# wolny/pytorch-3dunet

Measured on AMD Instinct MI355X. Metric: volumetric patches/sec (fwd+bwd), UNet3D f_maps=32 patch 64x128x128, higher is better.
Workload: dtype f32

## Files before the change

### pytorch-3dunet_amd/csrc/u3d_bf16.hip

```cpp
#include "u3d_common.h"
#include "u3d_gn.h"
#include <type_traits>

typedef __bf16 bf16x8 __attribute__((ext_vector_type(8)));
typedef __bf16 bf16x4 __attribute__((ext_vector_type(4)));
typedef __bf16 bf16x2 __attribute__((ext_vector_type(2)));
typedef float f32x2 __attribute__((ext_vector_type(2)));
typedef unsigned u32x4 __attribute__((ext_vector_type(4)));
typedef unsigned u32x2 __attribute__((ext_vector_type(2)));

__device__ __forceinline__ bf16x8 u3d_stage_b16(const bf16x8& v, bool has_aff, bool ok, const f32x4& a0, const f32x4& b0, const f32x4& a1,
                                                const f32x4& b1) {
    const u32x4 raw = __builtin_bit_cast(u32x4, v);
    u32x4 o = raw;
    if (has_aff) {
#pragma unroll
        for (int e = 0; e < 4; ++e) {
            const f32x2 x = {__builtin_bit_cast(float, raw[e] << 16), __builtin_bit_cast(float, raw[e] & 0xffff0000u)};
            const f32x2 a = e < 2 ? f32x2{a0[2 * e], a0[2 * e + 1]} : f32x2{a1[2 * e - 4], a1[2 * e - 3]};
            const f32x2 b = e < 2 ? f32x2{b0[2 * e], b0[2 * e + 1]} : f32x2{b1[2 * e - 4], b1[2 * e - 3]};
            o[e] = __builtin_bit_cast(unsigned, __builtin_convertvector(__builtin_elementwise_fma(x, a, b), bf16x2));
        }
    }
    const unsigned m = ok ? 0xffffffffu : 0u;
    return __builtin_bit_cast(bf16x8, u32x4{o[0] & m, o[1] & m, o[2] & m, o[3] & m});
}

extern int g_u3d_tune[24];

namespace {

constexpr int HS = 12;

struct bf16_conv_params {
    const float* x;
    const float* affine;
    const bf16x8* wpk;
    float* y;
    const float* residual;
    const float* gx;
    double* out_stats;
    double* gstats;
    int N, D, H, W, C, K, relu;
    int tz, ty, tx;
    int off;
    const float* maskx;
    int ksplit;
    float* ws;
    long long wpart;
    int order;
    int b16;
    int t8mode, t8cs;
};

template <int ZW, int KS>
struct tile_geom {
    static constexpr bool FLAT = ZW == 3;
    static constexpr int TZ = FLAT ? 5 : 4 * ZW, TY = FLAT ? 10 : 8, TX = FLAT ? 10 : 8;
    static constexpr int HZ = TZ + KS - 1, HY = TY + KS - 1, HX = TX + KS - 1, MT = FLAT ? 4 : 2 * ZW;
    static_assert(HX <= HS, "halo rows are HS records long");
    static constexpr int NTAPS = KS * KS * KS;
    static constexpr int RING = KS == 3 ? 9 : 8;
    static constexpr int BDIST = 6;
    static constexpr int ADIST = 2;
    static constexpr int PLANE = HZ * HY * HS * 16 + 64;
    static constexpr int BUF = 2 * PLANE;
    static constexpr int ITEMS = HZ * HY * HX * 4;
    static constexpr int ITERS = (ITEMS + 255) / 256;
    static constexpr int NPARTS = KS * KS;
    static constexpr int PER_PART = (ITERS + NPARTS - 1) / NPARTS;
    static constexpr int ITEMS8 = HZ * HY * HX * 2;
    static constexpr int ITERS8 = (ITEMS8 + 255) / 256;
    static constexpr int PER_PART8 = (ITERS8 + NPARTS - 1) / NPARTS;
};

template <int NT, int ZW, int KS, typename T = float>
__device__ __forceinline__ void conv_tile_epilogue(const bf16_conv_params& p, f32x16 (&acc)[tile_geom<ZW, KS>::MT][NT], char* lds, int n, int nb,
                                                   int split, int z0, int y0, int x0, int t, int lane, int w) {
    using G = tile_geom<ZW, KS>;
    const int col = lane & 31, half = lane >> 5;
    if (p.ksplit > 1) {
// ... 2760 lines not shown
```

### pytorch-3dunet_amd/csrc/u3d_conv.hip

```cpp
#include <type_traits>
#include <utility>

#include "u3d_common.h"
#include "u3d_gn.h"
#include "u3d_subpix.h"

int g_u3d_tune[24] = {0};

namespace cv {
constexpr int TZ = 4, TY = 8, TX = 8;
constexpr int HZ = TZ + 2, HY = TY + 2, HX = TX + 2;
constexpr int CC = 16;
constexpr int CS = 16;
constexpr int RS = HX * CS + 4;
constexpr int PS = HY * RS;
constexpr int TILE_FLOATS = HZ * PS + 4;
constexpr int CNT_OFF = 2 * TILE_FLOATS;
constexpr int RED_OFF = CNT_OFF + 16;
constexpr int LDS_FLOATS = RED_OFF + 4 * 3 * 32 * 2;
constexpr int NITEMS = HZ * HY * HX * (CC / 4);
constexpr int NIT = (NITEMS + 255) / 256;
constexpr int NSTEP = 27 * (CC / 8);
constexpr int NSTEP_PAIRY = 36 * (CC / 8);
constexpr int NSTEP_N16 = 27;
constexpr int ST0 = 30;
constexpr int ISTORE = 5;
constexpr int PACK_PAD = 5;
static_assert(2 * (NIT - 1) < ST0 - 8 && ST0 + NIT <= NSTEP, "prefetch schedule must fit the k-loop");
}

struct ConvParams {
    u3d_src_t src;
    u3d_src_t gx;
    const float* wp;
    float* out;
    double* out_stats;
    double* gstats;
    const float* res;
    int N, D, H, W, Cout;
    int nchunks, ncb, ntot;
    int tz, ty, tx;
    int relu, vec, has_gx, ovec;
    int total;
    int gx_x2;
    int stagger;
    int stat_reps;
    int zfast;
    int ksplit, cps;
    long long part_stride;
    long long* dbg;
    int oz0, oy0, ox0, oz1, oy1, ox1;
    int mz, my, mx;
};

#define U3D_DBG_STAMP(slot)                                                   \
    do {                                                                      \
        if constexpr (DBG) {                                                  \
            if (l == 0) dbgw[slot] = (long long)__builtin_readcyclecounter(); \
        }                                                                     \
    } while (0)
// ... 1018 lines not shown
                            }
                            if (v16 == 0) {
                                double* r = &red[(((T.n & 1) * NT) * 32 + 4 * kq + e) * 2];
                                __hip_atomic_fetch_add(r, (double)a, __ATOMIC_RELAXED, __HIP_MEMORY_SCOPE_WORKGROUP);
                                __hip_atomic_fetch_add(r + 1, (double)b2, __ATOMIC_RELAXED, __HIP_MEMORY_SCOPE_WORKGROUP);
                            }
                        }
                    } else {
                        const int cq_ = (l >> 2) & 7;
                        stat_reduce(sq1, sq2, T.n, 0, PAIRY ? 4 * (cq_ & 3) : 4 * cq_);
                    }
                    sq1 = f32x4{0.f, 0.f, 0.f, 0.f};
                    sq2 = f32x4{0.f, 0.f, 0.f, 0.f};
                }
            }
            flush_stats(T.n, T.cb);
        }
        if (!has_next_tile) break;
        if constexpr (!ZEROC) {
#pragma unroll
            for (int mt = 0; mt < MT; ++mt)
#pragma unroll
                for (int nt = 0; nt < NT; ++nt)
#pragma unroll
                    for (int r = 0; r < 16; ++r) acc[mt][nt][r] = 0.f;
        }
        wi = nwi;
        dT = dTN;
        T = TN;
        wq = wqn;
    }
    if constexpr (DBG) {
        if (l == 0) dbgw[4] = ntiles;
    }
    U3D_DBG_STAMP(6);
}

namespace wg {
constexpr int TZ = 2, TY = 8, TX = 8;
constexpr int HZ = TZ + 2, HY = TY + 2, HX = TX + 2;
constexpr int CC = 32;
constexpr int CSg = 32, RSg = HX * CSg, PSg = HY * RSg;
constexpr int G_FLOATS = HZ * PSg;
constexpr int TV = TZ * TY * TX;
constexpr int DZ_FLOATS = TV * 32;
constexpr int DUMMY_OFF = G_FLOATS + DZ_FLOATS;
constexpr int BUF_FLOATS = G_FLOATS + DZ_FLOATS + 4;
constexpr int LDS_FLOATS = 2 * BUF_FLOATS;
constexpr int NTHR = 512;
constexpr int NITEMS_G = HZ * HY * HX * (CC / 4);
constexpr int NIT_G = (NITEMS_G + NTHR - 1) / NTHR;
constexpr int NIT_DZ = TV * 8 / NTHR;
constexpr int MAX_MAP_INTS = 4096;
}

struct WgradParams {
    u3d_src_t src;
    const float* dz;
    float* partial;
    int N, D, H, W, Cout;
    int nchunks, nkb, S;
    int tz, ty, tx, ntiles, tps;
    int vec, dzvec;
    int bz0, by0, bx0, bz1, by1, bx1;
};

template <bool VEC, bool REG = false, bool PAIR = false>
__global__ __launch_bounds__(512, 2) void conv3d_wgrad_kernel(const WgradParams p) {
    using namespace wg;
    constexpr int NA = PAIR ? 4 : 7;
    extern __shared__ __attribute__((aligned(16))) float lds[];
    int* zmapl = reinterpret_cast<int*>(lds + 2 * BUF_FLOATS);
    __builtin_amdgcn_s_setprio(3);
    const int t = threadIdx.x;
    const int l = t & 63, i = l & 31, h = l >> 5;
    const int w = __builtin_amdgcn_readfirstlane(t >> 6);
    const int tg = w & 3, hf = w >> 2;

    const int logical = u3d_xcd_remap(blockIdx.x, gridDim.x);
    const int kb = logical % p.nkb;
    const int chunk = (logical / p.nkb) % p.nchunks;
    const int s = logical / (p.nkb * p.nchunks);
    const int D = p.D, H = p.H, W = p.W;
    const int Ctot = p.src.C0 + p.src.C1;
    int* ymapl = zmapl + D;
    int* xmapl = ymapl + H;
    if (p.src.C1 > 0) {
        for (int k = t; k < D; k += NTHR) zmapl[k] = p.src.zmap[k];
        for (int k = t; k < H; k += NTHR) ymapl[k] = p.src.ymap[k];
        for (int k = t; k < W; k += NTHR) xmapl[k] = p.src.xmap[k];
        __syncthreads();
    }

    f32x16 acc[NA];
#pragma unroll
    for (int k = 0; k < NA; ++k)
#pragma unroll
        for (int r = 0; r < 16; ++r) acc[k][r] = 0.f;

    const int q = t & 7, tv = t >> 3;
    const int cq = chunk * CC + 4 * q;
    const int co = kb * 32 + 4 * q;
    const bool cok = cq < Ctot, from0 = cq < p.src.C0, dcok = co < p.Cout;
    const float* gbase = !cok ? p.src.p0 : (from0 ? p.src.p0 + cq : p.src.p1 + (cq - p.src.C0));
    const int Cs = (from0 || !cok) ? p.src.C0 : p.src.C1;
    const float* dzbase = p.dz + (dcok ? co : 0);

    constexpr int NPFC = NIT_G + NIT_DZ;
    int rel[NPFC], loff[NPFC];
    unsigned fz0 = 0, fz1 = 0, fy0 = 0, fy1 = 0, fx0 = 0, fx1 = 0, fdead = 0;
    if constexpr (REG) {
        const int vz = D % TZ ? D % TZ : TZ, vy = H % TY ? H % TY : TY, vx = W % TX ? W % TX : TX;
#pragma unroll
        for (int it = 0; it < NIT_G; ++it) {
            const int vox = tv + 64 * it;
            const int hz = vox / (HY * HX);
            const int rem = vox - hz * (HY * HX);
            const int hy = rem / HX;
            const int hx = rem - hy * HX;
            const bool in = vox < HZ * HY * HX;
            rel[it] = from0 ? ((hz - 1) * H + (hy - 1)) * W + (hx - 1)
                            : (((hz - 1) >> 1) * p.src.H1 + ((hy - 1) >> 1)) * p.src.W1 + ((hx - 1) >> 1);
            loff[it] = in ? hz * PSg + hy * RSg + hx * CSg + 4 * q : DUMMY_OFF;
            fz0 |= (in && hz == 0 ? 1u : 0u) << it;
            fz1 |= (in && hz > vz ? 1u : 0u) << it;
            fy0 |= (in && hy == 0 ? 1u : 0u) << it;
            fy1 |= (in && hy > vy ? 1u : 0u) << it;
            fx0 |= (in && hx == 0 ? 1u : 0u) << it;
            fx1 |= (in && hx > vx ? 1u : 0u) << it;
            fdead |= (in && cok ? 0u : 1u) << it;
        }
#pragma unroll
        for (int it = 0; it < NIT_DZ; ++it) {
            const int vox = tv + 64 * it;
            rel[NIT_G + it] = ((vox >> 6) * H + ((vox >> 3) & 7)) * W + (vox & 7);
            loff[NIT_G + it] = G_FLOATS + vox * 32 + 4 * q;
            fz1 |= ((vox >> 6) >= vz ? 1u : 0u) << (NIT_G + it);
            fy1 |= (((vox >> 3) & 7) >= vy ? 1u : 0u) << (NIT_G + it);
            fx1 |= ((vox & 7) >= vx ? 1u : 0u) << (NIT_G + it);
        }
        fdead |= (dcok ? 0u : 3u) << NIT_G;
    }
    auto tile_invalid = [&](int z0, int y0, int x0) {
        unsigned inv = fdead;
        inv |= z0 == 0 ? fz0 : 0u;
        inv |= z0 + TZ >= D ? fz1 : 0u;
        inv |= y0 == 0 ? fy0 : 0u;
        inv |= y0 + TY >= H ? fy1 : 0u;
        inv |= x0 == 0 ? fx0 : 0u;
        inv |= x0 + TX >= W ? fx1 : 0u;
        return inv;
// ... 124 lines not shown
        f32x4 ga, gb;
        u3d_load_affine(p.src.affine, c.n, Ctot, cq, false, ga, gb);
#pragma unroll 1
        for (int it = 0; it < NIT_G; ++it) {
            const int vox = tv + 64 * it;
            if (vox >= HZ * HY * HX) continue;
            const int hz = vox / (HY * HX), rem = vox - hz * (HY * HX), hy = rem / HX, hx = rem - hy * HX;
            const int gz = c.z0 - 1 + hz, gy = c.y0 - 1 + hy, gxx = c.x0 - 1 + hx;
            f32x4 val = {0.f, 0.f, 0.f, 0.f};
            if (gz >= 0 && gz < D && gy >= 0 && gy < H && gxx >= 0 && gxx < W) {
                int v0, v1;
                u3d_vox_index(p.src, c.n, gz, gy, gxx, D, H, W, v0, v1);
                val = u3d_load_quad(p.src, v0, v1, cq, false) * ga + gb;
            }
            *reinterpret_cast<f32x4*>(&buf[hz * PSg + hy * RSg + hx * CSg + 4 * q]) = val;
        }
#pragma unroll 1
        for (int it = 0; it < NIT_DZ; ++it) {
            const int vox = tv + 64 * it;
            const int z = c.z0 + (vox >> 6), y = c.y0 + ((vox >> 3) & 7), x = c.x0 + (vox & 7);
            f32x4 val = {0.f, 0.f, 0.f, 0.f};
            if (z < p.bz1 && y < p.by1 && x < p.bx1) {
                const float* sp = p.dz + ((size_t)((c.n * D + z) * H + y) * W + x) * p.Cout + co;
#pragma unroll
                for (int e = 0; e < 4; ++e)
                    if (co + e < p.Cout) val[e] = sp[e];
            }
            *reinterpret_cast<f32x4*>(&buf[G_FLOATS + vox * 32 + 4 * q]) = val;
        }
    };

    constexpr int NPF = NIT_G + NIT_DZ;
    constexpr int ST0 = 20;
    static_assert(2 * (NPF - 1) < ST0 && ST0 + NPF <= 32, "prefetch schedule must fit the 32 groups of a tile");
    const int tile_begin = s * p.tps, tile_end = min(p.ntiles, (s + 1) * p.tps);

    TileIdx tix = tile_decode(tile_begin);
    if (tile_begin < tile_end) {
        const TileC c = tile_coords(tix);
        if constexpr (VEC) {
            f32x4 ga, gb;
            load_affine(c.n, ga, gb);
            f32x4 v[NPF];
#pragma unroll
            for (int k = 0; k < NPF; ++k) v[k] = pf_load(c, k);
#pragma unroll
            for (int k = 0; k < NPF; ++k) pf_store(lds, c, k, v[k], ga, gb);
        } else {
            stage_scalar(lds, c);
        }
    }
    __syncthreads();

    int abase[NA];
#pragma unroll
    for (int k = 0; k < NA; ++k) {
        const int tap = PAIR ? 2 * (tg + 4 * k) + (i >> 4) : tg + 4 * k;
        const int toff = tap < 27 ? (tap / 9) * PSg + ((tap / 3) % 3) * RSg + (tap % 3) * CSg : 0;
        abase[k] = (PAIR ? (i & 15) : i) + h * CSg + hf * PSg + toff;
    }
    int bbase = G_FLOATS + (hf * 64 + h) * 32 + i;
    int cur = 0;
    __builtin_amdgcn_s_setprio(0);

    f32x4 gan = {1.f, 1.f, 1.f, 1.f}, gbn = {0.f, 0.f, 0.f, 0.f};
    int n_aff = -1;
    for (int tile = tile_begin; tile < tile_end; ++tile) {
        const bool has_next = tile + 1 < tile_end;
        if (has_next) tix = tile_next(tix);
        const TileC cn = tile_coords(tix);
        float* nbuf = lds + (cur ^ 1) * BUF_FLOATS;
        f32x4 v[NPF];
        if constexpr (VEC) {
            if (cn.n != n_aff) {
                load_affine(cn.n, gan, gbn);
                n_aff = cn.n;
            }
        }
        const float* gl = lds + cur * BUF_FLOATS;

        float aop[2][NA], bop[2];
        bop[0] = gl[bbase];
#pragma unroll
        for (int k = 0; k < NA; ++k) aop[0][k] = gl[abase[k]];
#pragma unroll
        for (int g = 0; g < 32; ++g) {
            if constexpr (VEC) {
                if (g % 2 == 0 && g / 2 < NPF) v[g / 2] = pf_load(cn, g / 2);
                if (g >= ST0 && g - ST0 < NPF) pf_store(nbuf, cn, g - ST0, v[g - ST0], gan, gbn);
            }
            if (g + 1 < 32) {
                const int row = (g + 1) >> 2, tq = (g + 1) & 3;
                const int goff = row * RSg + 2 * tq * CSg;
                bop[(g + 1) & 1] = gl[bbase + (row * 8 + 2 * tq) * 32];
#pragma unroll
                for (int k = 0; k < NA; ++k) aop[(g + 1) & 1][k] = gl[abase[k] + goff];
            }
            __builtin_amdgcn_sched_barrier(0);
#pragma unroll
            for (int k = 0; k < NA; ++k) acc[k] = __builtin_amdgcn_mfma_f32_32x32x2f32(aop[g & 1][k], bop[g & 1], acc[k], 0, 0, 0);
            __builtin_amdgcn_sched_barrier(0);
        }
        if constexpr (!VEC) {
            if (has_next) stage_scalar(nbuf, cn);
        }
        __syncthreads();
        cur ^= 1;
    }

    __builtin_amdgcn_s_setprio(3);
    float* red = lds;
    if (hf == 1) {
#pragma unroll
        for (int k = 0; k < NA; ++k)
#pragma unroll
            for (int r = 0; r < 16; ++r) red[((tg * 7 + k) * 16 + r) * 64 + l] = acc[k][r];
    }
    __syncthreads();
    if (hf == 0) {
        float* dst = p.partial + ((size_t)((s * p.nchunks + chunk) * p.nkb + kb) * 27) * 1024;
#pragma unroll
        for (int k = 0; k < NA; ++k) {
#pragma unroll
            for (int r = 0; r < 16; ++r) {
                const int row = (r & 3) + 8 * (r >> 2) + 4 * h;
                const int tap = PAIR ? 2 * (tg + 4 * k) + (row >> 4) : tg + 4 * k;
                const int c = PAIR ? (row & 15) : row;
                if (tap < 27) dst[((size_t)tap * 32 + c) * 32 + i] = acc[k][r] + red[((tg * 7 + k) * 16 + r) * 64 + l];
            }
        }
    }
}

template <int G>
__global__ __launch_bounds__(256) void wgrad_reduce_kernel(const float* __restrict__ partial, float* __restrict__ dw,
                                                           int S, int nchunks, int nkb, int Cin, int Cout, int cstride,
                                                           int has_job, u3d_gn_bwd_job_t job) {
    __shared__ float red[4][64];
    if (has_job && blockIdx.x == 0) {
        extern __shared__ double shb[];
        u3d_gn_bwd_finalize_body(job.gstats_lo, job.mean_rstd, job.gamma, job.N, job.C0 + job.C1, job.G, job.count, 1, 1, job.dgamma,
                                 job.dbeta, job.coef, job.gstats_hi, job.C0, job.hi_scale, job.coef_hi, shb, job.reps_lo, job.reps_hi);
        return;
    }
    const long long total = (long long)Cin * 27 * Cout;
    const int lane = G == 1 ? (int)threadIdx.x : (int)(threadIdx.x & 63), grp = G == 1 ? 0 : (int)(threadIdx.x >> 6);
    const long long idx = (long long)(blockIdx.x - (has_job ? 1 : 0)) * (G == 1 ? 256 : 64) + lane;
    float sum = 0.f;
    int k = 0, tap = 0, c = 0;
    if (idx < total) {
        k = (int)(idx % Cout);
        const long long r = idx / Cout;
        tap = (int)(r % 27);
        c = (int)(r / 27);
        const int chunk = c >> 5, kb = k >> 5;
        const size_t off = ((size_t)(chunk * nkb + kb) * 27 + tap) * 1024 + (c & 31) * 32 + (k & 31);
        const size_t sstride = (size_t)nchunks * nkb * 27 * 1024;
        const int per = (S + G - 1) / G;
        const int s0 = grp * per, s1 = min(S, s0 + per);
        float a0 = 0.f, a1 = 0.f, a2 = 0.f, a3 = 0.f;
        int s = s0;
        for (; s + 3 < s1; s += 4) {
            a0 += partial[(size_t)s * sstride + off];
            a1 += partial[(size_t)(s + 1) * sstride + off];
            a2 += partial[(size_t)(s + 2) * sstride + off];
            a3 += partial[(size_t)(s + 3) * sstride + off];
        }
        for (; s < s1; ++s) a0 += partial[(size_t)s * sstride + off];
        sum = (a0 + a1) + (a2 + a3);
    }
    if constexpr (G == 1) {
        if (idx < total) dw[((size_t)k * cstride + c) * 27 + tap] = sum;
    } else {
        red[grp][lane] = sum;
        __syncthreads();
        if (grp == 0 && idx < total)
            dw[((size_t)k * cstride + c) * 27 + tap] = (red[0][lane] + red[1][lane]) + (red[2][lane] + red[3][lane]);
    }
}

__device__ __forceinline__ int pack_image_of(long long idx, int nchunks, int ntot, long long& id) {
// ... 299 lines not shown
        v /= H;
        const int z = (int)(v % D);
        const int n = (int)(v / D);
        float sum = 0.f;
        for (int tap = 0; tap < 27; ++tap) {
            const int zz = z + tap / 9 - 1, yy = y + (tap / 3) % 3 - 1, xx = x + tap % 3 - 1;
            if (zz < 0 || zz >= D || yy < 0 || yy >= H || xx < 0 || xx >= W) continue;
            int v0, v1;
            u3d_vox_index(src, n, zz, yy, xx, D, H, W, v0, v1);
            for (int c = 0; c < Cin; ++c) {
                float g = u3d_load_elem(src, v0, v1, c);
                if (src.affine) {
                    const float* ab = src.affine + ((size_t)n * Cin + c) * 2;
                    g = g * ab[0] + ab[1];
                }
                const float wt = flip ? w[((size_t)c * Cout + co) * 27 + (26 - tap)] : w[((size_t)co * Cin + c) * 27 + tap];
                sum += g * wt;
            }
        }
        if (relu) sum = fmaxf(sum, 0.f);
        out[idx] = sum;
    }
}

static inline int cdiv(int a, int b) { return (a + b - 1) / b; }

static bool src_vec_ok(const u3d_src_t* s) {
    if (s->C0 % 4 != 0 || s->C1 % 4 != 0) return false;
    if (((uintptr_t)s->p0 & 15) != 0) return false;
    if (s->C1 > 0 && ((uintptr_t)s->p1 & 15) != 0) return false;
    if (s->affine && ((uintptr_t)s->affine & 15) != 0) return false;
    return true;
}

static int check_src(const u3d_src_t* s, const char* what) {
    U3D_REQUIRE(s != nullptr && s->p0 != nullptr && (s->C0 > 0 || s->C1 > 0) && s->C0 >= 0, "%s: null source", what);
    U3D_REQUIRE(s->C1 >= 0, "%s: negative C1", what);
    if (s->C1 > 0)
        U3D_REQUIRE(s->p1 && s->zmap && s->ymap && s->xmap && s->D1 > 0 && s->H1 > 0 && s->W1 > 0,
                    "%s: low-res source needs p1, index maps and dims", what);
    return 0;
}

static long long* g_u3d_prof_buf = nullptr;
static size_t g_u3d_prof_records = 0;

extern "C" int u3d_set_profile_buffer(void* device_buffer, size_t bytes) {
    g_u3d_prof_buf = static_cast<long long*>(device_buffer);
    g_u3d_prof_records = device_buffer ? bytes / (24 * sizeof(long long)) : 0;
    return 0;
}

extern "C" int u3d_set_tuning(int key, int value) {
    if (key < 0 || key >= 24) return u3d_set_err(U3D_EINVAL, "u3d_set_tuning: key out of range");
    g_u3d_tune[key] = value;
    return 0;
}

extern "C" size_t u3d_packed_weight_floats(int Cin, int Cout, int mode) {
    return (size_t)pack_total_floats(Cin, Cout, mode, nullptr, nullptr);
}

extern "C" int u3d_pack_weights(int device, u3d_stream_t stream, const float* w, int Cout, int Cin, int mode,
                                float* packed) {
    U3D_ENTER(device);
    U3D_REQUIRE(w && packed && Cout > 0 && Cin > 0 && (mode == 0 || mode == 1), "u3d_pack_weights: bad argument");
    int nchunks = 0, ntot = 0;
    const long long total = pack_total_floats(Cin, Cout, mode, &nchunks, &ntot);
    const int blocks = (int)((total + 255) / 256 > 4096 ? 4096 : (total + 255) / 256);
    hipLaunchKernelGGL(pack_weights_kernel, dim3(blocks), dim3(256), 0, (hipStream_t)stream, w, packed, Cout, Cin,
                       mode, nchunks, ntot, total);
    U3D_LAUNCH_CHECK();
    return 0;
}

extern "C" int u3d_pack_weights_batch(int device, u3d_stream_t stream, const u3d_pack_desc_t* descs_device, int n,
                                      int64_t total_floats) {
    U3D_ENTER(device);
    U3D_REQUIRE(descs_device && n > 0 && total_floats > 0, "u3d_pack_weights_batch: bad argument");
    U3D_REQUIRE(total_floats % 4 == 0, "u3d_pack_weights_batch: image sizes are multiples of 4 floats");
    long long blocks = (total_floats / 4 + 255) / 256;
    if (blocks > 8192) blocks = 8192;
    hipLaunchKernelGGL(pack_weights_batch_kernel, dim3((unsigned)blocks), dim3(256), 0, (hipStream_t)stream, descs_device, n,
                       (long long)total_floats);
    U3D_LAUNCH_CHECK();
    return 0;
}

extern "C" long long u3d_pack_weights_cells_blocks(const float* w, int Cin, int Cout, int mode, int cin_stride) {
    const int cs = cin_stride > 0 ? cin_stride : Cin;
    if (Cin <= 0 || Cout <= 0 || mode < 0 || mode > 3 || Cin % 4 != 0 || Cout % 4 != 0 || cs % 4 != 0 || ((uintptr_t)w & 15) != 0) return 0;
    return pack_cells_of(Cin, Cout, mode) + 1;
}

extern "C" int u3d_pack_weights_batch_cells(int device, u3d_stream_t stream, const u3d_pack_desc_t* descs_device, int n,
                                            long long total_blocks) {
    U3D_ENTER(device);
    U3D_REQUIRE(descs_device && n > 0 && total_blocks > 0 && total_blocks < 0x7fffffffLL, "u3d_pack_weights_batch_cells: bad argument");
    hipLaunchKernelGGL(pack_weights_cells_kernel, dim3((unsigned)total_blocks), dim3(256), 0, (hipStream_t)stream, descs_device, n);
    U3D_LAUNCH_CHECK();
    return 0;
}

static int device_cu_count(int device, int* out) {
    static int cached[64] = {0};
    if (device >= 0 && device < 64 && cached[device] > 0) {
        *out = cached[device];
// ... 350 lines not shown
        else                                                                                     \
            hipLaunchKernelGGL((conv3d_mfma_kernel<NT_, false>), grid, block, shmem, st, p);     \
    } while (0)
    if (nt == 3)
        U3D_CONV_LAUNCH(3);
    else if (nt == 2)
        U3D_CONV_LAUNCH(2);
    else
        U3D_CONV_LAUNCH(1);
#undef U3D_CONV_LAUNCH
    U3D_LAUNCH_CHECK();
    return 0;
}

static void wgrad_plan(int N, int D, int H, int W, int Cin, int Cout, WgradParams& p) {
    p.nchunks = cdiv(Cin, 32);
    p.nkb = cdiv(Cout, 32);
    p.tz = cdiv(D, wg::TZ), p.ty = cdiv(H, wg::TY), p.tx = cdiv(W, wg::TX);
    p.ntiles = N * p.tz * p.ty * p.tx;
    const int pairs = p.nchunks * p.nkb;
    const int ncu = 256;
    long long best_cost = -1;
    int best_S = 1;
    for (int rounds = 1; rounds <= 8; ++rounds) {
        int S = (rounds * ncu) / pairs;
        if (S < 1) S = 1;
        if (S > p.ntiles) S = p.ntiles;
        const int tps = cdiv(p.ntiles, S);
        S = cdiv(p.ntiles, tps);
        const long long cost = (long long)cdiv(S * pairs, ncu) * (tps + 2);
        if (best_cost < 0 || cost < best_cost) {
            best_cost = cost;
            best_S = S;
        }
    }
    if (g_u3d_tune[1] > 0) best_S = g_u3d_tune[1] > p.ntiles ? p.ntiles : g_u3d_tune[1];
    p.tps = cdiv(p.ntiles, best_S);
    p.S = cdiv(p.ntiles, p.tps);
}

extern "C" size_t u3d_wgrad_workspace_floats(int N, int D, int H, int W, int Cin, int Cout) {
    WgradParams p;
    wgrad_plan(N, D, H, W, Cin, Cout, p);
    return (size_t)p.S * p.nchunks * p.nkb * 27 * 1024;
}

static int wgrad_set_lds_once(int device) {
    static bool done[64] = {false};
    if (device >= 0 && device < 64 && done[device]) return 0;
    U3D_HIP(hipFuncSetAttribute(reinterpret_cast<const void*>(conv3d_wgrad_kernel<true, true>),
                                hipFuncAttributeMaxDynamicSharedMemorySize, (wg::LDS_FLOATS + wg::MAX_MAP_INTS) * sizeof(float)));
    U3D_HIP(hipFuncSetAttribute(reinterpret_cast<const void*>(conv3d_wgrad_kernel<true, true, true>),
                                hipFuncAttributeMaxDynamicSharedMemorySize, (wg::LDS_FLOATS + wg::MAX_MAP_INTS) * sizeof(float)));
    U3D_HIP(hipFuncSetAttribute(reinterpret_cast<const void*>(conv3d_wgrad_kernel<true>),
                                hipFuncAttributeMaxDynamicSharedMemorySize, (wg::LDS_FLOATS + wg::MAX_MAP_INTS) * sizeof(float)));
    U3D_HIP(hipFuncSetAttribute(reinterpret_cast<const void*>(conv3d_wgrad_kernel<false>),
                                hipFuncAttributeMaxDynamicSharedMemorySize, (wg::LDS_FLOATS + wg::MAX_MAP_INTS) * sizeof(float)));
    if (device >= 0 && device < 64) done[device] = true;
    return 0;
}

static int conv3d_wgrad_impl(int device, u3d_stream_t stream, const u3d_src_t* src, const float* dz, float* dw, int cstride,
                             int N, int D, int H, int W, int Cout, float* workspace, size_t workspace_floats, const int* box = nullptr,
                             const u3d_gn_bwd_job_t* job = nullptr);

extern "C" int u3d_conv3d_wgrad_box(int device, u3d_stream_t stream, const u3d_src_t* src, const float* dz, float* dw, int N, int D,
                                    int H, int W, int Cout, float* workspace, size_t workspace_floats, const int* box) {
    U3D_REQUIRE(box != nullptr, "u3d_conv3d_wgrad_box: box is NULL");
    return conv3d_wgrad_impl(device, stream, src, dz, dw, 0, N, D, H, W, Cout, workspace, workspace_floats, box);
}

extern "C" int u3d_conv3d_wgrad(int device, u3d_stream_t stream, const u3d_src_t* src, const float* dz, float* dw,
                                int N, int D, int H, int W, int Cout, float* workspace, size_t workspace_floats) {
    return conv3d_wgrad_impl(device, stream, src, dz, dw, 0, N, D, H, W, Cout, workspace, workspace_floats);
}

extern "C" int u3d_conv3d_wgrad_strided(int device, u3d_stream_t stream, const u3d_src_t* src, const float* dz, float* dw,
                                        int dw_cin_stride, int N, int D, int H, int W, int Cout, float* workspace,
                                        size_t workspace_floats) {
    U3D_REQUIRE(src && dw_cin_stride >= src->C0 + src->C1, "u3d_conv3d_wgrad_strided: dw_cin_stride < channels of src");
    return conv3d_wgrad_impl(device, stream, src, dz, dw, dw_cin_stride, N, D, H, W, Cout, workspace, workspace_floats);
}

static size_t wgrad_job_lds_bytes(int N, int C, int G) { return sizeof(double) * (4 * (size_t)N * C + 2 * (size_t)N * G); }

extern "C" int u3d_conv3d_wgrad_job_supported(int N, int C, int G) {
    return (N > 0 && C > 0 && G > 0 && C % G == 0 && wgrad_job_lds_bytes(N, C, G) + 1024 <= 64 * 1024) ? 1 : 0;
}

extern "C" int u3d_conv3d_wgrad_job(int device, u3d_stream_t stream, const u3d_src_t* src, const float* dz, float* dw,
                                    int dw_cin_stride, int N, int D, int H, int W, int Cout, float* workspace,
                                    size_t workspace_floats, const u3d_gn_bwd_job_t* job) {
    U3D_REQUIRE(src && (dw_cin_stride == 0 || dw_cin_stride >= src->C0 + src->C1), "u3d_conv3d_wgrad_job: dw_cin_stride < channels of src");
    if (job) {
        U3D_REQUIRE(job->gstats_lo && job->mean_rstd && job->gamma && job->dgamma && job->dbeta && job->coef && job->C0 > 0 &&
                        job->C1 >= 0 && (job->C1 == 0) == (job->gstats_hi == nullptr) && (job->coef_hi == nullptr || job->C1 > 0) &&
                        job->reps_lo >= 0 && job->reps_lo <= 64 && job->reps_hi >= 0 && job->reps_hi <= 64,
                    "u3d_conv3d_wgrad_job: bad job");
        U3D_REQUIRE(u3d_conv3d_wgrad_job_supported(job->N, job->C0 + job->C1, job->G) == 1,
                    "u3d_conv3d_wgrad_job: the reduction of %d x %d channels in %d groups does not fit one block's LDS", job->N,
                    job->C0 + job->C1, job->G);
    }
    return conv3d_wgrad_impl(device, stream, src, dz, dw, dw_cin_stride, N, D, H, W, Cout, workspace, workspace_floats, nullptr, job);
}

static int conv3d_wgrad_impl(int device, u3d_stream_t stream, const u3d_src_t* src, const float* dz, float* dw, int cstride,
                             int N, int D, int H, int W, int Cout, float* workspace, size_t workspace_floats, const int* box,
                             const u3d_gn_bwd_job_t* job) {
    U3D_ENTER(device);
    if (int e = check_src(src, "u3d_conv3d_wgrad")) return e;
    U3D_REQUIRE(dz && dw && workspace && N > 0 && D > 0 && H > 0 && W > 0 && Cout > 0, "u3d_conv3d_wgrad: bad argument");
    U3D_REQUIRE((long long)N * D * H * W < (1ll << 31), "u3d_conv3d_wgrad: N*D*H*W must be < 2^31");
    WgradParams p;
    const int Cin = src->C0 + src->C1;
    p.bz0 = p.by0 = p.bx0 = 0, p.bz1 = D, p.by1 = H, p.bx1 = W;
    if (box) {
        U3D_REQUIRE(box[0] >= 0 && box[1] >= 0 && box[2] >= 0 && box[3] <= D && box[4] <= H && box[5] <= W && box[0] < box[3] &&
                        box[1] < box[4] && box[2] < box[5], "u3d_conv3d_wgrad_box: box outside the volume or empty");
        p.bz0 = box[0], p.by0 = box[1], p.bx0 = box[2], p.bz1 = box[3], p.by1 = box[4], p.bx1 = box[5];
    }
    wgrad_plan(N, p.bz1 - p.bz0, p.by1 - p.by0, p.bx1 - p.bx0, Cin, Cout, p);
    const size_t need = (size_t)p.S * p.nchunks * p.nkb * 27 * 1024;
    if (workspace_floats < need)
        return u3d_set_err(U3D_EWORKSPACE, "u3d_conv3d_wgrad: workspace %zu < %zu floats", workspace_floats, need);
    p.src = *src;
    p.dz = dz;
    p.partial = workspace;
    p.N = N, p.D = D, p.H = H, p.W = W, p.Cout = Cout;
    p.vec = src_vec_ok(src) ? 1 : 0;
    p.dzvec = (Cout % 4 == 0 && ((uintptr_t)dz & 15) == 0) ? 1 : 0;
    if (int e = wgrad_set_lds_once(device)) return e;
    const int nblk = p.S * p.nchunks * p.nkb;
    U3D_REQUIRE(D + H + W <= wg::MAX_MAP_INTS, "u3d_conv3d_wgrad: D+H+W must be <= %d", wg::MAX_MAP_INTS);
    const size_t shmem = (wg::LDS_FLOATS + (size_t)(D + H + W)) * sizeof(float);
    const bool reg = !box && (g_u3d_tune[3] != 2 || (D % wg::TZ == 0 && H % wg::TY == 0 && W % wg::TX == 0)) &&
                     (src->C1 == 0 || (D == 2 * src->D1 && H == 2 * src->H1 && W == 2 * src->W1));
    if (p.vec && p.dzvec && reg && Cin <= 16)
        hipLaunchKernelGGL((conv3d_wgrad_kernel<true, true, true>), dim3(nblk), dim3(wg::NTHR), shmem, (hipStream_t)stream, p);
    else if (p.vec && p.dzvec && reg)
        hipLaunchKernelGGL((conv3d_wgrad_kernel<true, true>), dim3(nblk), dim3(wg::NTHR), shmem, (hipStream_t)stream, p);
    else if (p.vec && p.dzvec)
        hipLaunchKernelGGL(conv3d_wgrad_kernel<true>, dim3(nblk), dim3(wg::NTHR), shmem, (hipStream_t)stream, p);
    else
        hipLaunchKernelGGL(conv3d_wgrad_kernel<false>, dim3(nblk), dim3(wg::NTHR), shmem, (hipStream_t)stream, p);
    U3D_LAUNCH_CHECK();
    const long long total = (long long)Cin * 27 * Cout;
    const bool one_group = p.S <= 16 && g_u3d_tune[23] != 1;
    const int rblocks = (int)((total + (one_group ? 255 : 63)) / (one_group ? 256 : 64));
    u3d_gn_bwd_job_t jb = {};
    size_t job_lds = 0;
    if (job) {
        jb = *job;
        if (!jb.gstats_hi) jb.C1 = 0, jb.hi_scale = 1.0f, jb.coef_hi = nullptr;
        if (jb.reps_lo < 1) jb.reps_lo = 1;
        if (jb.reps_hi < 1 || !jb.gstats_hi) jb.reps_hi = 1;
        job_lds = wgrad_job_lds_bytes(jb.N, jb.C0 + jb.C1, jb.G);
    }
    if (one_group)
        hipLaunchKernelGGL(wgrad_reduce_kernel<1>, dim3(rblocks + (job ? 1 : 0)), dim3(256), job_lds, (hipStream_t)stream, workspace, dw, p.S,
                           p.nchunks, p.nkb, Cin, Cout, cstride > 0 ? cstride : Cin, job ? 1 : 0, jb);
    else
        hipLaunchKernelGGL(wgrad_reduce_kernel<4>, dim3(rblocks + (job ? 1 : 0)), dim3(256), job_lds, (hipStream_t)stream, workspace, dw, p.S,
                           p.nchunks, p.nkb, Cin, Cout, cstride > 0 ? cstride : Cin, job ? 1 : 0, jb);
    U3D_LAUNCH_CHECK();
    return 0;
}

extern "C" int u3d_conv3d_variant(int N, int D, int H, int W, int Cin, int Cout, int src_kind, int has_workspace) {
    if (N <= 0 || D <= 0 || H <= 0 || W <= 0 || Cin <= 0 || Cout <= 0) return -1;
    if (Cin % 4 != 0 || Cout % 4 != 0) return 0;
    const long long ntiles = (long long)N * cdiv(D, cv::TZ) * cdiv(H, cv::TY) * cdiv(W, cv::TX);
    const int nchunks = cdiv(Cin, 16), ntot = cdiv(Cout, 32);
    if (has_workspace && splitk_shape(N, D, H, W, Cin, Cout) && g_u3d_tune[7] != 2) {
        if (splitk_count(g_u3d_ncu_seen, ntiles, ntot, nchunks, nullptr) >= 2) return 3;
    }
    const bool ragged = D % cv::TZ != 0 || H % cv::TY != 0 || W % cv::TX != 0;
    if (src_kind == 2 || g_u3d_tune[3] == 1 || (g_u3d_tune[3] == 2 && ragged)) return 0;
    return ragged ? 2 : 1;
}

extern "C" int u3d_conv3d_wgrad_variant(int N, int D, int H, int W, int Cin, int Cout, int src_kind) {
    if (N <= 0 || D <= 0 || H <= 0 || W <= 0 || Cin <= 0 || Cout <= 0) return -1;
    if (Cin % 4 != 0 || Cout % 4 != 0) return 0;
    const bool ragged = D % wg::TZ != 0 || H % wg::TY != 0 || W % wg::TX != 0;
    if (src_kind == 2 || (g_u3d_tune[3] == 2 && ragged)) return 0;
    return (ragged ? 2 : 1) | (Cin <= 16 ? 4 : 0);
}

extern "C" int u3d_conv3d_naive(int device, u3d_stream_t stream, const u3d_src_t* src, const float* w, float* out,
                                int N, int D, int H, int W, int Cin, int Cout, int relu, int flip) {
// ... 11 lines not shown
```

### pytorch-3dunet_amd/csrc/u3d_ops.hip

```cpp
#include "u3d_common.h"
#include "u3d_gn.h"

#include <string.h>

extern int g_u3d_tune[24];

static thread_local char g_err[512] = "";

int u3d_set_err(int code, const char* fmt, ...) {
    va_list ap;
    va_start(ap, fmt);
    vsnprintf(g_err, sizeof(g_err), fmt, ap);
    va_end(ap);
    return code;
}

int u3d_device_guard::enter(int device) {
    hipError_t e = hipGetDevice(&prev);
    if (e != hipSuccess) return u3d_set_err(U3D_EHIP, "hipGetDevice failed: %s", hipGetErrorString(e));
    if (device >= 0 && prev != device) {
        e = hipSetDevice(device);
        if (e != hipSuccess) return u3d_set_err(U3D_EHIP, "hipSetDevice(%d) failed: %s", device, hipGetErrorString(e));
        switched = true;
    }
    return 0;
}

extern "C" int u3d_version(void) { return U3D_VERSION; }
extern "C" const char* u3d_last_error(void) { return g_err; }

extern "C" int u3d_check_device(int device) {
    hipDeviceProp_t prop;
    U3D_HIP(hipGetDeviceProperties(&prop, device));
    if (strncmp(prop.gcnArchName, "gfx950", 6) != 0)
        return u3d_set_err(U3D_EARCH, "device %d is %s, this library is built for gfx950 only", device, prop.gcnArchName);
    return 0;
}

__global__ __launch_bounds__(256) void debug_stream_pass_kernel(float* __restrict__ buf, long long n4, int passes, float one,
                                                               long long ticks_total) {
    f32x4* b = reinterpret_cast<f32x4*>(buf);
    constexpr long long PIECE = 4096;
    const long long npieces = (n4 + PIECE - 1) / PIECE;
    const long long mine = (npieces - blockIdx.x + gridDim.x - 1) / gridDim.x;
    const long long t0 = wall_clock64();
    long long done = 0;
    for (int p = 0; p < passes; ++p)
        for (long long pc = blockIdx.x; pc < npieces; pc += gridDim.x) {
            const long long lo = pc * PIECE, hi = lo + PIECE < n4 ? lo + PIECE : n4;
            for (long long i = lo + threadIdx.x; i < hi; i += 256) {
                f32x4 v = b[i];
                v *= one;
                b[i] = v;
            }
            ++done;
            if (ticks_total > 0) {
                const long long due = t0 + ticks_total * done / (mine * passes);
                while (wall_clock64() < due) __builtin_amdgcn_s_sleep(64);
// ... 1855 lines not shown
```

### pytorch-3dunet_amd/csrc/u3d_smallc.hip

```cpp
#include "u3d_common.h"

extern int g_u3d_tune[24];

typedef float f32x4s __attribute__((ext_vector_type(4)));

namespace sc {
constexpr int TZ = 4, TY = 8, TX = 8;
constexpr int HZ = 6, HY = 10, HX = 10;
constexpr int HV = HZ * HY * HX;
constexpr int MAXC = 4;
}

struct SmallFwdParams {
    const float* x;
    const float* affine;
    const float* w;
    float* out;
    double* out_stats;
    int N, D, H, W, Cin, Cout, relu;
    int tz, ty, tx, B;
    int reps;
};

template <int COUTP>
__global__ __launch_bounds__(256) void conv3d_small_fwd_kernel(const SmallFwdParams p) {
    using namespace sc;
    __shared__ __attribute__((aligned(16))) float xs[HV * MAXC];
    __shared__ __attribute__((aligned(16))) float ws[27 * MAXC * COUTP];
    __shared__ double sred[COUTP][2];
    const int t = threadIdx.x;
    const int n = blockIdx.y;
    const int Cin = p.Cin, D = p.D, H = p.H, W = p.W;
    for (int i = t; i < 27 * Cin * COUTP; i += 256) {
        const int k = i % COUTP;
        const int r = i / COUTP;
        const int c = r % Cin, tap = r / Cin;
        ws[i] = k < p.Cout ? p.w[((size_t)k * Cin + c) * 27 + tap] : 0.f;
    }
    if (t < COUTP) sred[t][0] = sred[t][1] = 0.0;
    float s1[COUTP], s2[COUTP];
#pragma unroll
    for (int k = 0; k < COUTP; ++k) s1[k] = s2[k] = 0.f;
    const int zl = t >> 6, yl = (t >> 3) & 7, xl = t & 7;
    const int ntiles = p.tz * p.ty * p.tx;
    for (int tile = blockIdx.x; tile < ntiles; tile += p.B) {
        int tt = tile;
        const int txi = tt % p.tx;
        tt /= p.tx;
        const int tyi = tt % p.ty;
        const int tzi = tt / p.ty;
        const int z0 = tzi * TZ, y0 = tyi * TY, x0 = txi * TX;
        __syncthreads();
        for (int i = t; i < HV * Cin; i += 256) {
            const int c = i % Cin;
            const int hv = i / Cin;
// ... 593 lines not shown
```

### pytorch-3dunet_amd/csrc/u3d_subpix.hip

```cpp
#include "u3d_subpix.h"

extern int g_u3d_tune[24];


struct SubpixParams {
    const float* low;
    const float* affine;
    long long aff_nstride;
    const float* wp;
    float* out;
    int N, D1, H1, W1, C1, Cout, Do, Ho, Wo;
    int tz, ty, tx, nchunks, ncb;
    int ksplit, cps;
    long long part_stride;
    int oz, oy, ox;
};

__device__ __forceinline__ void sp_flag_signal(int* c, int lane) {
    asm volatile("" ::: "memory");
    if (lane == 0) __hip_atomic_fetch_add(c, 1, __ATOMIC_RELAXED, __HIP_MEMORY_SCOPE_WORKGROUP);
    asm volatile("" ::: "memory");
}
__device__ __forceinline__ void sp_flag_wait(int* c, int target) {
    while (__hip_atomic_load(c, __ATOMIC_RELAXED, __HIP_MEMORY_SCOPE_WORKGROUP) < target) __builtin_amdgcn_s_sleep(2);
    asm volatile("" ::: "memory");
}

template <class S>
__global__ __launch_bounds__(256, 2) void subpixel_fwd_kernel(const SubpixParams p) {
    using namespace sp;
    using SC = Sch<S>;
    constexpr int NFRAG = NFRAG_OF<S>, RING = S::RING, NACT = NACT_OF<S>;
    constexpr int LE = NACT >= 2 * NIT + 8 ? 2 : 1;
    constexpr int KS0 = NACT >= 40 ? 30 : NACT - NIT - 1;
    constexpr int KA = KS0 >= 6 ? KS0 - 6 : 0;
    static_assert(LE * (NIT - 1) < KS0 && KS0 + NIT <= NACT, "prefetch schedule must fit the k-loop");
    __shared__ __attribute__((aligned(16))) float lds[2 * TILE_FLOATS];
    __shared__ int cnt[16];
    const int t = threadIdx.x;
    const int l = t & 63, w = t >> 6, m = l & 31, h = l >> 5;
    __builtin_amdgcn_s_setprio(3);
    if (t < 16) cnt[t] = 0;
    __syncthreads();

    int logical = u3d_xcd_remap(blockIdx.x, gridDim.x);
    int ch0 = 0, nch = p.nchunks;
    float* const outp = p.out + (size_t)(p.ksplit > 1 ? logical % p.ksplit : 0) * p.part_stride;
    if (p.ksplit > 1) {
        ch0 = (logical % p.ksplit) * p.cps;
        nch = min(p.cps, p.nchunks - ch0);
        logical /= p.ksplit;
    }
    const int cb = logical % p.ncb;
    int tile = logical / p.ncb;
    const int txi = tile % p.tx;
// ... 991 lines not shown
```

Measured before the change: 120.9.

## Add 16x16x4 MFMA wgrad variant for small-channel inputs with balanced tap units

Adds a C16 specialisation of the weight-gradient kernel for Cin<=16 that uses 16x16x4 f32 MFMA instead of 32x32x2 with paired taps. Work is split into (tap, column-half) units distributed across waves with a compile-time checked table, so each SIMD gets 27 units. This is meant to avoid the padding waste of the PAIR scheme, where 32-row MFMA tiles were half used for 16-channel inputs. In exchange, a wave issues more, smaller MFMA instructions, and the reduction and store paths change. It is the new default, with a tuning key to fall back.

```diff
diff --git a/pytorch-3dunet_amd/csrc/u3d_bf16.hip b/pytorch-3dunet_amd/csrc/u3d_bf16.hip
--- a/pytorch-3dunet_amd/csrc/u3d_bf16.hip
+++ b/pytorch-3dunet_amd/csrc/u3d_bf16.hip
@@ -26,7 +26,7 @@
     return __builtin_bit_cast(bf16x8, u32x4{o[0] & m, o[1] & m, o[2] & m, o[3] & m});
 }
 
-extern int g_u3d_tune[24];
+extern int g_u3d_tune[25];
 
 namespace {
 
diff --git a/pytorch-3dunet_amd/csrc/u3d_conv.hip b/pytorch-3dunet_amd/csrc/u3d_conv.hip
--- a/pytorch-3dunet_amd/csrc/u3d_conv.hip
+++ b/pytorch-3dunet_amd/csrc/u3d_conv.hip
@@ -5,7 +5,7 @@
 #include "u3d_gn.h"
 #include "u3d_subpix.h"
 
-int g_u3d_tune[24] = {0};
+int g_u3d_tune[25] = {0};
 
 namespace cv {
 constexpr int TZ = 4, TY = 8, TX = 8;
@@ -1130,6 +1130,28 @@
 constexpr int NIT_G = (NITEMS_G + NTHR - 1) / NTHR;
 constexpr int NIT_DZ = TV * 8 / NTHR;
 constexpr int MAX_MAP_INTS = 4096;
+
+namespace c16 {
+constexpr int MAXU = 14;
+constexpr int order(int tg, int hf) { return hf ? 3 - tg : tg; }
+constexpr int first_tap(int o) { return o < 2 ? 7 * o : 14 + 6 * (o - 2); }
+constexpr int units(int o) { return o < 2 ? 14 : 13; }
+constexpr int unit_tap(int o, int u) { return (u < 12 || o < 2) ? first_tap(o) + u / 2 : 26; }
+constexpr int unit_half(int o, int u) { return (u & 1) ^ (o == 3 ? 1 : 0); }
+constexpr bool table_ok() {
+    for (int hf = 0; hf < 2; ++hf) {
+        int seen[54] = {};
+        for (int tg = 0; tg < 4; ++tg)
+            for (int u = 0; u < units(order(tg, hf)); ++u) seen[2 * unit_tap(order(tg, hf), u) + unit_half(order(tg, hf), u)] += 1;
+        for (int k = 0; k < 54; ++k)
+            if (seen[k] != 1) return false;
+    }
+    for (int tg = 0; tg < 4; ++tg)
+        if (units(order(tg, 0)) + units(order(tg, 1)) != 27) return false;
+    return true;
+}
+static_assert(table_ok(), "every (tap, column half) once per voxel half, 27 units per SIMD");
+}
 }
 
 struct WgradParams {
@@ -1143,10 +1165,14 @@
     int bz0, by0, bx0, bz1, by1, bx1;
 };
 
-template <bool VEC, bool REG = false, bool PAIR = false>
+template <bool VEC, bool REG = false, bool PAIR = false, bool C16 = false>
 __global__ __launch_bounds__(512, 2) void conv3d_wgrad_kernel(const WgradParams p) {
     using namespace wg;
-    constexpr int NA = PAIR ? 4 : 7;
+    static_assert(!C16 || (VEC && REG && !PAIR), "the 16-column variant exists for constant-offset staging only");
+    constexpr int NA = C16 ? c16::MAXU : (PAIR ? 4 : 7);
+    constexpr int NR = C16 ? 4 : 16;
+    constexpr int NAOP = C16 ? 7 : NA;
+    using acc_t = std::conditional_t<C16, f32x4, f32x16>;
     extern __shared__ __attribute__((aligned(16))) float lds[];
     int* zmapl = reinterpret_cast<int*>(lds + 2 * BUF_FLOATS);
     __builtin_amdgcn_s_setprio(3);
@@ -1170,11 +1196,11 @@
         __syncthreads();
     }
 
-    f32x16 acc[NA];
+    acc_t acc[NA];
 #pragma unroll
     for (int k = 0; k < NA; ++k)
 #pragma unroll
-        for (int r = 0; r < 16; ++r) acc[k][r] = 0.f;
+        for (int r = 0; r < NR; ++r) acc[k][r] = 0.f;
 
     const int q = t & 7, tv = t >> 3;
     const int cq = chunk * CC + 4 * q;
@@ -1405,14 +1431,19 @@
     }
     __syncthreads();
 
-    int abase[NA];
-#pragma unroll
-    for (int k = 0; k < NA; ++k) {
-        const int tap = PAIR ? 2 * (tg + 4 * k) + (i >> 4) : tg + 4 * k;
+    const int ord = c16::order(tg, hf), i16 = l & 15, kq = l >> 4;
+    int abase[NAOP];
+#pragma unroll
+    for (int k = 0; k < NAOP; ++k) {
+        const int tap = C16 ? c16::unit_tap(ord, 2 * k) : (PAIR ? 2 * (tg + 4 * k) + (i >> 4) : tg + 4 * k);
         const int toff = tap < 27 ? (tap / 9) * PSg + ((tap / 3) % 3) * RSg + (tap % 3) * CSg : 0;
-        abase[k] = (PAIR ? (i & 15) : i) + h * CSg + hf * PSg + toff;
+        abase[k] = C16 ? i16 + kq * CSg + hf * PSg + toff
+                       : (PAIR ? (i & 15) : i) + h * CSg + hf * PSg + toff;
     }
     int bbase = G_FLOATS + (hf * 64 + h) * 32 + i;
+    int bbase16[2];
+#pragma unroll
+    for (int j = 0; j < 2; ++j) bbase16[j] = G_FLOATS + (hf * 64 + kq) * 32 + 16 * c16::unit_half(ord, j) + i16;
     int cur = 0;
     __builtin_amdgcn_s_setprio(0);
 
@@ -1432,27 +1463,57 @@
         }
         const float* gl = lds + cur * BUF_FLOATS;
 
-        float aop[2][NA], bop[2];
-        bop[0] = gl[bbase];
-#pragma unroll
-        for (int k = 0; k < NA; ++k) aop[0][k] = gl[abase[k]];
-#pragma unroll
-        for (int g = 0; g < 32; ++g) {
+        auto stage_step = [&](int g) {
             if constexpr (VEC) {
                 if (g % 2 == 0 && g / 2 < NPF) v[g / 2] = pf_load(cn, g / 2);
                 if (g >= ST0 && g - ST0 < NPF) pf_store(nbuf, cn, g - ST0, v[g - ST0], gan, gbn);
             }
-            if (g + 1 < 32) {
-                const int row = (g + 1) >> 2, tq = (g + 1) & 3;
-                const int goff = row * RSg + 2 * tq * CSg;
-                bop[(g + 1) & 1] = gl[bbase + (row * 8 + 2 * tq) * 32];
-#pragma unroll
-                for (int k = 0; k < NA; ++k) aop[(g + 1) & 1][k] = gl[abase[k] + goff];
-            }
-            __builtin_amdgcn_sched_barrier(0);
-#pragma unroll
-            for (int k = 0; k < NA; ++k) acc[k] = __builtin_amdgcn_mfma_f32_32x32x2f32(aop[g & 1][k], bop[g & 1], acc[k], 0, 0, 0);
-            __builtin_amdgcn_sched_barrier(0);
+        };
+        if constexpr (C16) {
+            float aop[2][NAOP], bop[2][2];
+#pragma unroll
+            for (int j = 0; j < 2; ++j) bop[0][j] = gl[bbase16[j]];
+#pragma unroll
+            for (int k = 0; k < NAOP; ++k) aop[0][k] = gl[abase[k]];
+#pragma unroll
+            for (int qd = 0; qd < 16; ++qd) {
+                stage_step(2 * qd);
+                stage_step(2 * qd + 1);
+                if (qd + 1 < 16) {
+                    const int row = (qd + 1) >> 1, xq = (qd + 1) & 1;
+#pragma unroll
+                    for (int j = 0; j < 2; ++j) bop[(qd + 1) & 1][j] = gl[bbase16[j] + (row * 8 + 4 * xq) * 32];
+#pragma unroll
+                    for (int k = 0; k < NAOP; ++k) aop[(qd + 1) & 1][k] = gl[abase[k] + row * RSg + 4 * xq * CSg];
+                }
+                __builtin_amdgcn_sched_barrier(0);
+#pragma unroll
+                for (int u = 0; u < c16::MAXU - 1; ++u)
+                    acc[u] = __builtin_amdgcn_mfma_f32_16x16x4f32(aop[qd & 1][u / 2], bop[qd & 1][u & 1], acc[u], 0, 0, 0);
+                if (ord < 2)
+                    acc[c16::MAXU - 1] = __builtin_amdgcn_mfma_f32_16x16x4f32(aop[qd & 1][6], bop[qd & 1][1], acc[c16::MAXU - 1], 0, 0, 0);
+                __builtin_amdgcn_sched_barrier(0);
+            }
+        } else {
+            float aop[2][NA], bop[2];
+            bop[0] = gl[bbase];
+#pragma unroll
+            for (int k = 0; k < NA; ++k) aop[0][k] = gl[abase[k]];
+#pragma unroll
+            for (int g = 0; g < 32; ++g) {
+                stage_step(g);
+                if (g + 1 < 32) {
+                    const int row = (g + 1) >> 2, tq = (g + 1) & 3;
+                    const int goff = row * RSg + 2 * tq * CSg;
+                    bop[(g + 1) & 1] = gl[bbase + (row * 8 + 2 * tq) * 32];
+#pragma unroll
+                    for (int k = 0; k < NA; ++k) aop[(g + 1) & 1][k] = gl[abase[k] + goff];
+                }
+                __builtin_amdgcn_sched_barrier(0);
+#pragma unroll
+                for (int k = 0; k < NA; ++k) acc[k] = __builtin_amdgcn_mfma_f32_32x32x2f32(aop[g & 1][k], bop[g & 1], acc[k], 0, 0, 0);
+                __builtin_amdgcn_sched_barrier(0);
+            }
         }
         if constexpr (!VEC) {
             if (has_next) stage_scalar(nbuf, cn);
@@ -1463,23 +1524,50 @@
 
     __builtin_amdgcn_s_setprio(3);
     float* red = lds;
-    if (hf == 1) {
-#pragma unroll
-        for (int k = 0; k < NA; ++k)
-#pragma unroll
-            for (int r = 0; r < 16; ++r) red[((tg * 7 + k) * 16 + r) * 64 + l] = acc[k][r];
-    }
-    __syncthreads();
-    if (hf == 0) {
-        float* dst = p.partial + ((size_t)((s * p.nchunks + chunk) * p.nkb + kb) * 27) * 1024;
-#pragma unroll
-        for (int k = 0; k < NA; ++k) {
-#pragma unroll
-            for (int r = 0; r < 16; ++r) {
-                const int row = (r & 3) + 8 * (r >> 2) + 4 * h;
-                const int tap = PAIR ? 2 * (tg + 4 * k) + (row >> 4) : tg + 4 * k;
-                const int c = PAIR ? (row & 15) : row;
-                if (tap < 27) dst[((size_t)tap * 32 + c) * 32 + i] = acc[k][r] + red[((tg * 7 + k) * 16 + r) * 64 + l];
+    if constexpr (C16) {
+        const int nu = c16::units(ord);
+        if (hf == 1) {
+#pragma unroll
+            for (int u = 0; u < c16::MAXU; ++u) {
+                const int unit = 2 * c16::unit_tap(ord, u) + c16::unit_half(ord, u);
+                if (u < nu) {
+#pragma unroll
+                    for (int r = 0; r < 4; ++r) red[(unit * 4 + r) * 64 + l] = acc[u][r];
+                }
+            }
+        }
+        __syncthreads();
+        if (hf == 0) {
+            float* dst = p.partial + ((size_t)((s * p.nchunks + chunk) * p.nkb + kb) * 27) * 1024;
+#pragma unroll
+            for (int u = 0; u < c16::MAXU; ++u) {
+                const int tap = c16::unit_tap(ord, u), half = c16::unit_half(ord, u);
+                if (u < nu) {
+#pragma unroll
+                    for (int r = 0; r < 4; ++r)
+                        dst[((size_t)tap * 32 + 4 * kq + r) * 32 + 16 * half + i16] = acc[u][r] + red[((2 * tap + half) * 4 + r) * 64 + l];
+                }
+            }
+        }
+    } else {
+        if (hf == 1) {
+#pragma unroll
+            for (int k = 0; k < NA; ++k)
+#pragma unroll
+                for (int r = 0; r < 16; ++r) red[((tg * 7 + k) * 16 + r) * 64 + l] = acc[k][r];
+        }
+        __syncthreads();
+        if (hf == 0) {
+            float* dst = p.partial + ((size_t)((s * p.nchunks + chunk) * p.nkb + kb) * 27) * 1024;
+#pragma unroll
+            for (int k = 0; k < NA; ++k) {
+#pragma unroll
+                for (int r = 0; r < 16; ++r) {
+                    const int row = (r & 3) + 8 * (r >> 2) + 4 * h;
+                    const int tap = PAIR ? 2 * (tg + 4 * k) + (row >> 4) : tg + 4 * k;
+                    const int c = PAIR ? (row & 15) : row;
+                    if (tap < 27) dst[((size_t)tap * 32 + c) * 32 + i] = acc[k][r] + red[((tg * 7 + k) * 16 + r) * 64 + l];
+                }
             }
         }
     }
@@ -1885,7 +1973,7 @@
 }
 
 extern "C" int u3d_set_tuning(int key, int value) {
-    if (key < 0 || key >= 24) return u3d_set_err(U3D_EINVAL, "u3d_set_tuning: key out of range");
+    if (key < 0 || key >= 25) return u3d_set_err(U3D_EINVAL, "u3d_set_tuning: key out of range");
     g_u3d_tune[key] = value;
     return 0;
 }
@@ -2342,6 +2430,8 @@
                                 hipFuncAttributeMaxDynamicSharedMemorySize, (wg::LDS_FLOATS + wg::MAX_MAP_INTS) * sizeof(float)));
     U3D_HIP(hipFuncSetAttribute(reinterpret_cast<const void*>(conv3d_wgrad_kernel<true, true, true>),
                                 hipFuncAttributeMaxDynamicSharedMemorySize, (wg::LDS_FLOATS + wg::MAX_MAP_INTS) * sizeof(float)));
+    U3D_HIP(hipFuncSetAttribute(reinterpret_cast<const void*>(conv3d_wgrad_kernel<true, true, false, true>),
+                                hipFuncAttributeMaxDynamicSharedMemorySize, (wg::LDS_FLOATS + wg::MAX_MAP_INTS) * sizeof(float)));
     U3D_HIP(hipFuncSetAttribute(reinterpret_cast<const void*>(conv3d_wgrad_kernel<true>),
                                 hipFuncAttributeMaxDynamicSharedMemorySize, (wg::LDS_FLOATS + wg::MAX_MAP_INTS) * sizeof(float)));
     U3D_HIP(hipFuncSetAttribute(reinterpret_cast<const void*>(conv3d_wgrad_kernel<false>),
@@ -2425,7 +2515,9 @@
     const size_t shmem = (wg::LDS_FLOATS + (size_t)(D + H + W)) * sizeof(float);
     const bool reg = !box && (g_u3d_tune[3] != 2 || (D % wg::TZ == 0 && H % wg::TY == 0 && W % wg::TX == 0)) &&
                      (src->C1 == 0 || (D == 2 * src->D1 && H == 2 * src->H1 && W == 2 * src->W1));
-    if (p.vec && p.dzvec && reg && Cin <= 16)
+    if (p.vec && p.dzvec && reg && Cin <= 16 && g_u3d_tune[24] != 1)
+        hipLaunchKernelGGL((conv3d_wgrad_kernel<true, true, false, true>), dim3(nblk), dim3(wg::NTHR), shmem, (hipStream_t)stream, p);
+    else if (p.vec && p.dzvec && reg && Cin <= 16)
         hipLaunchKernelGGL((conv3d_wgrad_kernel<true, true, true>), dim3(nblk), dim3(wg::NTHR), shmem, (hipStream_t)stream, p);
     else if (p.vec && p.dzvec && reg)
         hipLaunchKernelGGL((conv3d_wgrad_kernel<true, true>), dim3(nblk), dim3(wg::NTHR), shmem, (hipStream_t)stream, p);
diff --git a/pytorch-3dunet_amd/csrc/u3d_ops.hip b/pytorch-3dunet_amd/csrc/u3d_ops.hip
--- a/pytorch-3dunet_amd/csrc/u3d_ops.hip
+++ b/pytorch-3dunet_amd/csrc/u3d_ops.hip
@@ -3,7 +3,7 @@
 
 #include <string.h>
 
-extern int g_u3d_tune[24];
+extern int g_u3d_tune[25];
 
 static thread_local char g_err[512] = "";
 
diff --git a/pytorch-3dunet_amd/csrc/u3d_smallc.hip b/pytorch-3dunet_amd/csrc/u3d_smallc.hip
--- a/pytorch-3dunet_amd/csrc/u3d_smallc.hip
+++ b/pytorch-3dunet_amd/csrc/u3d_smallc.hip
@@ -1,6 +1,6 @@
 #include "u3d_common.h"
 
-extern int g_u3d_tune[24];
+extern int g_u3d_tune[25];
 
 typedef float f32x4s __attribute__((ext_vector_type(4)));
 
diff --git a/pytorch-3dunet_amd/csrc/u3d_subpix.hip b/pytorch-3dunet_amd/csrc/u3d_subpix.hip
--- a/pytorch-3dunet_amd/csrc/u3d_subpix.hip
+++ b/pytorch-3dunet_amd/csrc/u3d_subpix.hip
@@ -1,6 +1,6 @@
 #include "u3d_subpix.h"
 
-extern int g_u3d_tune[24];
+extern int g_u3d_tune[25];
 
 
 struct SubpixParams {
```

After: 121.3 (median of 6 runs). Within noise of the previous version (+0.3%).
